# lrjconan/LanczosNetwork

Measured on NVIDIA H100. Metric: QM8 molecules/sec (forward), higher is better.
Workload: dtype f32

## Files before the change

lanczosnetwork_b200/csrc/filter_mlp_chain.cu:

```cuda
#include "tc_gemm.cuh"

namespace {

constexpr int S0MAX = 8;

struct ChainPolicy {
  static constexpr int kStagesB = 2;
  static constexpr int kStagesA = 4;
  struct Params {
    const float* table;
    const int32_t* rowmap;
    const int32_t* nrows;
    const float* W_hi;
    const float* W_lo;
    const float* bias_all;
    float* coeff;
    int Rall, L, S, Hd;
    int dbg;
  };
  static __device__ __forceinline__ bool mma0(const Params& p) { return p.S > S0MAX; }
  static __device__ __forceinline__ int first_stage(const Params& p) { return mma0(p) ? 0 : 1; }
  static __device__ __forceinline__ int steps_per_item(const Params& p) { return mma0(p) ? 4 : 2; }
  static __device__ __forceinline__ int rows(const Params& p) { return p.nrows ? __ldg(p.nrows) : p.Rall; }
  static __device__ __forceinline__ int ntile(const Params& p) { return (rows(p) + tcg::BM - 1) / tcg::BM; }
  static __device__ __forceinline__ void item_range(const Params& p, int cta, int ncta, int& first,
                                                    int& count) {
    const int items = ntile(p) * p.L, base = items / ncta, rem = items % ncta;
    count = base + (cta < rem ? 1 : 0);
    first = cta * base + min(cta, rem);
  }
  static __device__ __forceinline__ int num_steps(const Params& p, int cta, int ncta) {
    int first, count;
    item_range(p, cta, ncta, first, count);
    return count * steps_per_item(p);
  }
  static __device__ __forceinline__ void decode(const Params& p, int cta, int ncta, int it,
                                                int& m_tile, int& sub) {
    const int per = steps_per_item(p), nt = ntile(p);
    int first, count;
    item_range(p, cta, ncta, first, count);
    const int item = first + it / per;
    m_tile = item % nt;
    sub = (item / nt) * 4 + first_stage(p) + it % per;
  }
  static __device__ __forceinline__ int num_kblocks(const Params& p, int sub) {
    return (sub & 3) == 0 ? 1 : p.Hd / tcg::BK;
  }
  static __device__ __forceinline__ int w_row0(const Params& p, int layer, int stage) {
    return layer * (3 * p.Hd + p.S) + stage * p.Hd;
  }
  static __device__ __forceinline__ void w_coords(const Params& p, int sub, int kb, int& col0, int& row0) {
    col0 = kb * tcg::BK;
    row0 = w_row0(p, sub >> 2, sub & 3);
  }
  static __device__ __forceinline__ bool operand_from_acc(const Params& p, int sub) {
    return (sub & 3) > first_stage(p);
  }
  static __device__ __forceinline__ float acc_operand(const Params&, const uint8_t* policy_smem, int sub, int col,
                                                      float x) {
    const float* bs = reinterpret_cast<const float*>(policy_smem) + BS_OFF;
    return fmaxf(x + bs[(sub & 3) * tcg::BN + col], 0.f);
  }

  const Params& p;
  const int tid, r;
  static constexpr int BS_OFF = 2 * tcg::BN * S0MAX;
  float* W1s;
  float* W3s;
  float* bs;
  float* b3s;
  int src, cur_layer;
  float tv[S0MAX];
  float o[S0MAX];

  static size_t smem_bytes() {
    return (BS_OFF + 3 * tcg::BN + S0MAX) * 4;
  }

  __device__ ChainPolicy(const Params& p_, uint8_t* smem, int tid_)
      : p(p_), tid(tid_), r(tid_ & 127), src(-1), cur_layer(-1) {
    W1s = reinterpret_cast<float*>(smem);
    W3s = W1s + tcg::BN * S0MAX;
    bs = W1s + BS_OFF;
    b3s = bs + 3 * tcg::BN;
  }

  __device__ void step_begin(int m_tile, int sub, int, tcg::PhaseTimer& tm) {
    const int layer = sub >> 2;
    if ((sub & 3) != first_stage(p)) return;
    const int i = m_tile * tcg::BM + r;
    src = i < rows(p) ? (p.rowmap ? __ldg(p.rowmap + i) : i) : -1;
    if (layer != cur_layer) {
      tcg::producers_sync<ChainPolicy>();
      const int row0 = w_row0(p, layer, 0), row3 = w_row0(p, layer, 3);
      if (!mma0(p)) {
#pragma unroll 4
        for (int e = tid; e < p.Hd * S0MAX; e += tcg::producer_threads<ChainPolicy>) {
          const int c = e / S0MAX, k = e - c * S0MAX;
          const int64_t o1 = (int64_t)(row0 + c) * p.Hd + k;
          W1s[e] = (k < p.S) ? __ldg(p.W_hi + o1) + __ldg(p.W_lo + o1) : 0.f;
          const int64_t o3 = (int64_t)(row3 + k) * p.Hd + c;
          W3s[e] = (k < p.S) ? __ldg(p.W_hi + o3) + __ldg(p.W_lo + o3) : 0.f;
        }
        if (tid < S0MAX) b3s[tid] = tid < p.S ? __ldg(p.bias_all + row3 + tid) : 0.f;
      }
      for (int e = tid; e < 3 * tcg::BN; e += tcg::producer_threads<ChainPolicy>) {
        const int st = e / tcg::BN, c = e - st * tcg::BN;
        bs[e] = c < p.Hd ? __ldg(p.bias_all + row0 + st * p.Hd + c) : 0.f;
      }
      tcg::producers_sync<ChainPolicy>();
      cur_layer = layer;
      tm.lap(1);
    }
    if (mma0(p)) return;
#pragma unroll
    for (int k = 0; k < S0MAX; ++k)
      tv[k] = (src >= 0 && k < p.S) ? __ldg(p.table + (int64_t)src * p.S + k) : 0.f;
  }

  __device__ __forceinline__ void produce(int sub, int kb, float (&v)[32]) {
    if ((sub & 3) == 0) {
#pragma unroll
      for (int j = 0; j < 32; ++j)
        v[j] = (src >= 0 && j < p.S) ? __ldg(p.table + (int64_t)src * p.S + j) : 0.f;
      return;
    }
#pragma unroll
    for (int j = 0; j < 32; ++j) {
      const int c = kb * tcg::BK + j;
      const float4* wr = reinterpret_cast<const float4*>(W1s + c * S0MAX);
      const float4 wa = wr[0], wb = wr[1];
      float a = bs[c];
      a = fmaf(tv[0], wa.x, a); a = fmaf(tv[1], wa.y, a); a = fmaf(tv[2], wa.z, a); a = fmaf(tv[3], wa.w, a);
      a = fmaf(tv[4], wb.x, a); a = fmaf(tv[5], wb.y, a); a = fmaf(tv[6], wb.z, a); a = fmaf(tv[7], wb.w, a);
      v[j] = fmaxf(a, 0.f);
    }
  }
  __device__ __forceinline__ void pre_epilogue(int) {}
  __device__ __forceinline__ void post_epilogue(int) {}

  __device__ __forceinline__ void store(int sub, int col, const float (&x)[tcg::EW]) {
    const int layer = sub >> 2, stage = sub & 3;
    if (stage == 3) {
      if (src < 0 || col >= p.S) return;
      const float* bias = p.bias_all + w_row0(p, layer, stage);
      float* dst = p.coeff + ((int64_t)layer * p.Rall + src) * p.S;
#pragma unroll
      for (int j = 0; j < tcg::EW; ++j)
        if (col + j < p.S) dst[col + j] = x[j] + __ldg(bias + col + j);
      return;
    }
    if (col >= p.Hd) return;
    const float* b2 = bs + 2 * tcg::BN;
    if (col == 0) {
#pragma unroll
      for (int s = 0; s < S0MAX; ++s) o[s] = 0.f;
    }
#pragma unroll
    for (int j = 0; j < tcg::EW; ++j) {
      const float y = fmaxf(x[j] + b2[col + j], 0.f);
      const float4* wr = reinterpret_cast<const float4*>(W3s + (col + j) * S0MAX);
      const float4 wa = wr[0], wb = wr[1];
      o[0] = fmaf(y, wa.x, o[0]); o[1] = fmaf(y, wa.y, o[1]);
      o[2] = fmaf(y, wa.z, o[2]); o[3] = fmaf(y, wa.w, o[3]);
      o[4] = fmaf(y, wb.x, o[4]); o[5] = fmaf(y, wb.y, o[5]);
      o[6] = fmaf(y, wb.z, o[6]); o[7] = fmaf(y, wb.w, o[7]);
    }
    if (col + tcg::EW < p.Hd || src < 0) return;
    float* dst = p.coeff + ((int64_t)layer * p.Rall + src) * p.S;
#pragma unroll
    for (int s = 0; s < S0MAX; ++s)
      if (s < p.S) dst[s] = o[s] + b3s[s];
  }
};

__global__ void __launch_bounds__(1024)
ritz_rowmap_kernel(const int32_t* __restrict__ gext, int B, int K, int32_t* __restrict__ rowmap,
                   int32_t* __restrict__ nrows) {
  __shared__ int warp_sums[32];
  __shared__ int gbase[1024], gk[1024];
  __shared__ int running;
  const int tid = threadIdx.x, lane = tid & 31, warp = tid >> 5;
  if (tid == 0) running = 0;
  __syncthreads();
  for (int b0 = 0; b0 < B; b0 += 1024) {
    const int b = b0 + tid;
    int k = (b < B) ? min(gext[b * 2 + 1], K) : 0;
    int incl = k;
#pragma unroll
    for (int o = 1; o < 32; o <<= 1) {
      const int t = __shfl_up_sync(0xffffffffu, incl, o);
      if (lane >= o) incl += t;
    }
    if (lane == 31) warp_sums[warp] = incl;
    __syncthreads();
    if (warp == 0) {
      int w = warp_sums[lane], wi = w;
#pragma unroll
      for (int o = 1; o < 32; o <<= 1) {
        const int t = __shfl_up_sync(0xffffffffu, wi, o);
        if (lane >= o) wi += t;
      }
      warp_sums[lane] = wi - w;
    }
    __syncthreads();
    const int base = running + warp_sums[warp] + incl - k;
    gbase[tid] = base;
    gk[tid] = k;
    __syncthreads();
    if (tid == 1023) running = base + k;
    for (int j = warp; j < 1024 && b0 + j < B; j += 32)
      for (int i = lane; i < gk[j]; i += 32) rowmap[gbase[j] + i] = (b0 + j) * K + i;
    __syncthreads();
  }
  if (tid == 0) nrows[0] = running;
}

}

extern "C" {

int lnb_ritz_rowmap(lnb_stream_t stream, const int32_t* gext, int B, int K, int32_t* rowmap,
                    int32_t* nrows) {
  LNB_REQUIRE(gext && rowmap && nrows, "ritz_rowmap: null pointer");
  LNB_REQUIRE(B >= 0 && K >= 1, "ritz_rowmap: bad dims");
  ritz_rowmap_kernel<<<1, 1024, 0, (cudaStream_t)stream>>>(gext, B, K, rowmap, nrows);
  lnb::count_launch();
  return lnb::finish_launch("ritz_rowmap");
}

int lnb_ritz_filter_mlp(lnb_stream_t stream, const float* table, const int32_t* rowmap,
                        const int32_t* nrows, const float* W_hi, const float* W_lo,
                        const float* bias_all, int Rall, int L, int S, int Hd, float* coeff) {
  return lnb_ritz_filter_mlp_ctas(stream, table, rowmap, nrows, W_hi, W_lo, bias_all, Rall, L, S, Hd,
                                  coeff, 0);
}

int lnb_ritz_filter_mlp_ctas(lnb_stream_t stream, const float* table, const int32_t* rowmap,
                             const int32_t* nrows, const float* W_hi, const float* W_lo,
                             const float* bias_all, int Rall, int L, int S, int Hd, float* coeff,
                             int ctas) {
  LNB_REQUIRE(table && W_hi && W_lo && bias_all && coeff, "ritz_filter_mlp: null pointer");
  LNB_REQUIRE((rowmap == nullptr) == (nrows == nullptr), "ritz_filter_mlp: rowmap and nrows go together");
  LNB_REQUIRE(Rall >= 0 && L >= 1 && S >= 1 && Hd >= 1 && ctas >= 0, "ritz_filter_mlp: bad dims");
  if (S > 32 || Hd % 32 != 0 || Hd > tcg::BN) {
    lnb::set_err("ritz_filter_mlp: unsupported shape S=%d hidden=%d (needs S<=32, hidden%%32==0, hidden<=128)", S, Hd);
    return LNB_ERR_UNSUPPORTED;
  }
  if (Rall == 0) return LNB_OK;
  const size_t smem = tcg::core_smem(ChainPolicy::kStagesB, ChainPolicy::kStagesA) + 1024 + ChainPolicy::smem_bytes();
  ChainPolicy::Params p{table, rowmap, nrows, W_hi, W_lo, bias_all, coeff, Rall, L, S, Hd, tcg::debug_flags()};
  return tcg::launch<ChainPolicy>(stream, W_hi, W_lo, L * (3 * Hd + S), Hd, smem, lnb::ceil_div(Rall, tcg::BM) * L, p,
                                  "ritz_filter_mlp", ctas);
}

}
```

lanczosnetwork_b200/csrc/tc_gemm.cuh:

```cuda
#pragma once
#include "common.cuh"
#include "sm90.cuh"
#include <stdlib.h>
#include <type_traits>
#include <utility>

namespace tcg {

constexpr int BM = 128, BN = 128, BK = 32;
constexpr int TILE_B_BYTES = BN * BK * 4;
constexpr int STAGE_B_BYTES = 2 * TILE_B_BYTES;
constexpr int TILE_A_BYTES = BM * BK * 4;
constexpr int STAGE_A_BYTES = 2 * TILE_A_BYTES;
constexpr int EW = 16;
constexpr int CONSUMER_THREADS = 256;
constexpr int CONSUMER_REGS = 168;
constexpr int MAX_B_STAGES = 6, MAX_A_STAGES = 4;

template <class P, class = void> struct ProducerGroups : std::integral_constant<int, 1> {};
template <class P>
struct ProducerGroups<P, std::void_t<decltype(P::kProducerGroups)>> : std::integral_constant<int, P::kProducerGroups> {};
template <class P> constexpr int producer_threads = 128 * ProducerGroups<P>::value;
template <class P> constexpr int cta_threads = producer_threads<P> + CONSUMER_THREADS;
template <class P> constexpr int producer_regs = (65536 - CONSUMER_THREADS * CONSUMER_REGS) / producer_threads<P> / 8 * 8;
__host__ __device__ constexpr int core_smem(int stages_b, int stages_a) {
  return stages_b * STAGE_B_BYTES + stages_a * STAGE_A_BYTES + 256;
}
__host__ __device__ constexpr int pass_cols(int stages_a) {
  return stages_a * STAGE_A_BYTES / (BM * 4) < BN ? stages_a * STAGE_A_BYTES / (BM * 4) : BN;
}

__device__ __forceinline__ uint8_t* a_ring(uint8_t* policy_smem, int stages_b, int stages_a) {
  return policy_smem - core_smem(stages_b, stages_a) + stages_b * STAGE_B_BYTES;
}

struct Core {
  uint8_t* Bst;
  uint8_t* Ast;
  uint64_t* b_full;
  uint64_t* b_empty;
  uint64_t* a_full;
  uint64_t* a_empty;
  uint64_t* stg_full;
  uint64_t* stg_empty;
  uint64_t* kept_read;
};

__device__ __forceinline__ Core carve(uint8_t* base, int stages_b, int stages_a) {
  Core c;
  c.Bst = base;
  c.Ast = base + stages_b * STAGE_B_BYTES;
  uint64_t* bars = reinterpret_cast<uint64_t*>(c.Ast + stages_a * STAGE_A_BYTES);
  c.b_full = bars;
  c.b_empty = c.b_full + MAX_B_STAGES;
  c.a_full = c.b_empty + MAX_B_STAGES;
  c.a_empty = c.a_full + MAX_A_STAGES;
  c.stg_full = c.a_empty + MAX_A_STAGES;
  c.stg_empty = c.stg_full + 1;
  c.kept_read = c.stg_empty + 1;
  return c;
}

__device__ unsigned long long* g_prof = nullptr;

struct PhaseTimer {
  unsigned long long* buf;
  long long t0;
  __device__ __forceinline__ void start(int cta, int tid) {
    buf = (tid == 0 && g_prof) ? g_prof + cta * 32 : nullptr;
    if (buf) t0 = clock64();
  }
  __device__ __forceinline__ void start_if(int cta, bool owner) {
    buf = (owner && g_prof) ? g_prof + cta * 32 : nullptr;
    if (buf) t0 = clock64();
  }
  __device__ __forceinline__ void lap(int slot) {
    if (buf) { long long t = clock64(); atomicAdd(&buf[slot], (unsigned long long)(t - t0)); t0 = t; }
  }
};

template <class Policy>
__device__ __forceinline__ void producers_sync() {
  asm volatile("bar.sync 1, %0;" ::"n"(producer_threads<Policy>) : "memory");
}
__device__ __forceinline__ void consumers_sync() {
  asm volatile("bar.sync 2, %0;" ::"n"(CONSUMER_THREADS) : "memory");
}

__device__ __forceinline__ int stg_index(int row, int col, int pw) {
  return row * pw + ((((col >> 2) ^ row) & (pw / 4 - 1)) << 2) + (col & 3);
}

template <class P, class = void> struct HasAccInit : std::false_type {};
template <class P> struct HasAccInit<P, std::void_t<decltype(&P::acc_init)>> : std::true_type {};
template <class P, class = void> struct HasOperandFromAcc : std::false_type {};
template <class P> struct HasOperandFromAcc<P, std::void_t<decltype(&P::operand_from_acc)>> : std::true_type {};
template <class P>
constexpr bool kScaledProduce =
    std::is_same_v<decltype(std::declval<P&>().produce(0, 0, std::declval<float (&)[32]>())), float>;

template <class Policy>
__device__ __forceinline__ bool next_from_acc(const typename Policy::Params& p, int cta, int ncta, int it,
                                              int nsteps, int& nkb_next) {
  if (it + 1 >= nsteps) return false;
  int m_tile, sub;
  Policy::decode(p, cta, ncta, it + 1, m_tile, sub);
  nkb_next = Policy::num_kblocks(p, sub);
  return Policy::operand_from_acc(p, sub);
}

constexpr int SKIP_MMA = 2;
constexpr int SKIP_TMA = 4;

template <class Policy, int kSkip>
__device__ __forceinline__ void tc_gemm_body(const CUtensorMap& map_hi, const CUtensorMap& map_lo,
                                             const typename Policy::Params& p) {
  extern __shared__ __align__(16) uint8_t smem_raw[];
  const uint32_t pad = (1024u - (sm90::smem_u32(smem_raw) & 1023u)) & 1023u;
  uint8_t* base = smem_raw + pad;
  constexpr int SB = Policy::kStagesB, SA = Policy::kStagesA;
  static_assert(SB >= 1 && SB <= MAX_B_STAGES && SA >= 1 && SA <= MAX_A_STAGES, "ring depths");
  constexpr int PW = pass_cols(SA);
  constexpr int NPASS = BN / PW;
  constexpr bool kAccInit = HasAccInit<Policy>::value;
  static_assert(!kAccInit || NPASS == 1, "a drain kept in the A ring must fit it in one pass");
  constexpr bool kOpAcc = HasOperandFromAcc<Policy>::value;
  constexpr bool kQueue = !kAccInit;
  static_assert(!kOpAcc || SA * BK >= BN, "an operand written from the accumulators needs one A stage per k-block");
  constexpr int NG = ProducerGroups<Policy>::value, PT = producer_threads<Policy>;
  constexpr bool kScaled = kScaledProduce<Policy>;
  static_assert(NG == 1 || (NG == 2 && !kOpAcc && PW % (2 * EW) == 0), "two producer groups: no operand_from_acc");
  Core c = carve(base, SB, SA);
  uint8_t* policy_smem = base + core_smem(SB, SA);
  float* stg = reinterpret_cast<float*>(c.Ast);

  const int tid = threadIdx.x, warp = tid >> 5, lane = tid & 31;
  const int role = __shfl_sync(0xffffffffu, tid / 128, 0);
  const int cta = blockIdx.x, ncta = gridDim.x;
  const int nsteps = __shfl_sync(0xffffffffu, Policy::num_steps(p, cta, ncta), 0);
  unsigned long long prof_ns0 = 0;
  long long prof_c0 = 0;
  if (tid == 0 && g_prof) {
    asm volatile("mov.u64 %0, %globaltimer;" : "=l"(prof_ns0));
    prof_c0 = clock64();
  }

  if (warp == PT / 32 && lane == 0) {
    sm90::tma_prefetch_desc(&map_hi);
    sm90::tma_prefetch_desc(&map_lo);
    for (int s = 0; s < SB; ++s) {
      sm90::mbar_init(&c.b_full[s], 1);
      sm90::mbar_init(&c.b_empty[s], CONSUMER_THREADS / 32);
    }
    for (int s = 0; s < SA; ++s) {
      sm90::mbar_init(&c.a_full[s], PT / NG);
      sm90::mbar_init(&c.a_empty[s], CONSUMER_THREADS / 32);
    }
    sm90::mbar_init(c.stg_full, CONSUMER_THREADS);
    sm90::mbar_init(c.stg_empty, PT);
    sm90::mbar_init(c.kept_read, CONSUMER_THREADS / 32);
    sm90::fence_barrier_init();
  }
  __syncthreads();

  if (NG == 1 ? role == 0 : role < NG) {
    if constexpr (NG > 1) sm90::setmaxnreg_dec<producer_regs<Policy>>();
    const int r = tid & 127;
    const int grp = NG == 1 ? 0 : role;
    Policy pol(p, policy_smem, tid);
    uint32_t cnt = 0;
    uint32_t npass = 0;
    uint32_t nkept = 0;
    bool after_kept = false;
    for (int it = 0; it < nsteps; ++it) {
      int m_tile, sub;
      Policy::decode(p, cta, ncta, it, m_tile, sub);
      int nkb = Policy::num_kblocks(p, sub);
      bool kept = false, to_acc = false;
      if constexpr (kAccInit) kept = Policy::drain_kept(p, sub);
      if constexpr (kOpAcc) {
        if (Policy::operand_from_acc(p, sub)) nkb = 0;
        int nkb_next;
        to_acc = next_from_acc<Policy>(p, cta, ncta, it, nsteps, nkb_next);
      }
      PhaseTimer tm;
      tm.start(cta, tid);
      pol.step_begin(m_tile, sub, NG == 1 ? 0 : (int)((grp + NG - cnt % NG) % NG), tm);
      [[maybe_unused]] float v_kept[32];
      for (int kb = 0; kb < nkb; ++kb, ++cnt) {
        if constexpr (NG > 1) {
          if (cnt % NG != (uint32_t)grp) continue;
        }
        float v[32];
        [[maybe_unused]] float scale = 1.f;
        if (!(p.dbg & 8)) {
          if constexpr (kScaled) scale = pol.produce(sub, kb, v_kept);
          else pol.produce(sub, kb, v);
        }
        const uint32_t sa = cnt % SA;
        if (kAccInit && (NG == 1 ? kb == 0 : kb < NG) && after_kept) {
          sm90::mbar_wait(c.kept_read, nkept & 1u);
          if constexpr (NG == 1) ++nkept;
        }
        sm90::mbar_wait(&c.a_empty[sa], ((cnt / SA) & 1u) ^ 1u);
        if (!(p.dbg & 1)) {
          uint8_t* hi = c.Ast + sa * STAGE_A_BYTES + r * 128;
#pragma unroll
          for (int j = 0; j < 8; ++j) {
            if constexpr (kScaled) {
#pragma unroll
              for (int i = 4 * j; i < 4 * j + 4; ++i) v[i] = __fmul_rn(scale, v_kept[i]);
            }
            uint4 h, l;
            h.x = sm90::tf32_rna_bits(v[4 * j + 0]); h.y = sm90::tf32_rna_bits(v[4 * j + 1]);
            h.z = sm90::tf32_rna_bits(v[4 * j + 2]); h.w = sm90::tf32_rna_bits(v[4 * j + 3]);
            l.x = sm90::tf32_rna_bits(v[4 * j + 0] - __uint_as_float(h.x));
            l.y = sm90::tf32_rna_bits(v[4 * j + 1] - __uint_as_float(h.y));
            l.z = sm90::tf32_rna_bits(v[4 * j + 2] - __uint_as_float(h.z));
            l.w = sm90::tf32_rna_bits(v[4 * j + 3] - __uint_as_float(h.w));
            const int off = (j ^ (r & 7)) * 16;
            *reinterpret_cast<uint4*>(hi + off) = h;
            *reinterpret_cast<uint4*>(hi + TILE_A_BYTES + off) = l;
          }
        }
        sm90::fence_proxy_async();
        sm90::mbar_arrive(&c.a_full[sa]);
      }
      if constexpr (NG > 1) {
        if (kAccInit && after_kept) ++nkept;
      }
      tm.lap((sub & 1) ? 8 : 3);
      pol.pre_epilogue(sub);
      tm.lap(4);
#pragma unroll 1
      for (int q = 0; q < (kept || to_acc ? 0 : NPASS); ++q, ++npass) {
        sm90::mbar_wait(c.stg_full, npass & 1u);
        if (q == 0) tm.lap((sub & 1) ? 9 : 5);
#pragma unroll 1
        for (int col = q * PW + grp * EW; col < (q + 1) * PW; col += NG * EW) {
          float x[EW];
#pragma unroll
          for (int j = 0; j < EW; j += 4) {
            const float4 t = *reinterpret_cast<const float4*>(stg + stg_index(r, col - q * PW + j, PW));
            x[j] = t.x; x[j + 1] = t.y; x[j + 2] = t.z; x[j + 3] = t.w;
          }
          pol.store(sub, col, x);
        }
        sm90::mbar_arrive(c.stg_empty);
      }
      tm.lap(7);
      producers_sync<Policy>();
      pol.post_epilogue(sub);
      tm.lap(10);
      after_kept = kept;
    }
  } else {
    if constexpr (NG > 1) sm90::setmaxnreg_inc<CONSUMER_REGS>();
    const int wg = role - NG;
    const int wq = warp & 3;
    float d[128];
    uint32_t cnt = 0, npass = 0;
    uint32_t nacc = 0;
    bool after_kept = false;
    const int row0 = wg * 64 + wq * 16 + (lane >> 2), cl = 2 * (lane & 3);
    const bool w_issuer = warp == PT / 32;
    int l_it = 0, l_kb = 0, l_nkb = -1, l_sub = 0;
    uint32_t l_cnt = 0;
    auto load_next = [&]() {
      while (l_it < nsteps) {
        if (l_nkb < 0) {
          int mt;
          Policy::decode(p, cta, ncta, l_it, mt, l_sub);
          l_nkb = Policy::num_kblocks(p, l_sub);
        }
        if (l_kb < l_nkb) break;
        ++l_it; l_kb = 0; l_nkb = -1;
      }
      if (l_it >= nsteps) return;
      int col0, row0;
      Policy::w_coords(p, l_sub, l_kb, col0, row0);
      const uint32_t st = l_cnt % SB;
      sm90::mbar_wait_uniform(&c.b_empty[st], ((l_cnt / SB) & 1u) ^ 1u);
      uint8_t* dst = c.Bst + st * STAGE_B_BYTES;
      sm90::tma_load_2d_pair_elected<(kSkip & SKIP_TMA) != 0>(w_issuer, &c.b_full[st], STAGE_B_BYTES, dst, &map_hi,
                                                               dst + TILE_B_BYTES, &map_lo, col0, row0);
      ++l_kb; ++l_cnt;
    };
    auto release = [&](uint32_t sb_rel, bool a_stage, uint32_t sa_rel) {
      sm90::mbar_arrive_pred(&c.a_empty[sa_rel], a_stage && lane == 0);
      sm90::mbar_arrive_pred(&c.b_empty[sb_rel], lane == 0);
      load_next();
    };
    for (int i = 0; i < SB; ++i) load_next();
    for (int it = 0; it < nsteps; ++it) {
      int m_tile, sub;
      Policy::decode(p, cta, ncta, it, m_tile, sub);
      const int nkb = Policy::num_kblocks(p, sub);
      bool kept = false, from_acc = false, to_acc = false;
      int nkb_next = 0;
      if constexpr (kOpAcc) {
        from_acc = Policy::operand_from_acc(p, sub);
        to_acc = next_from_acc<Policy>(p, cta, ncta, it, nsteps, nkb_next);
      }
      if constexpr (kAccInit) {
        kept = Policy::drain_kept(p, sub);
        sm90::wgmma_fence_operand(d);
        if (!Policy::acc_init(p, policy_smem, stg, sub, row0, cl, d)) {
#pragma unroll
          for (int i = 0; i < 128; ++i) d[i] = 0.f;
        }
        if (after_kept) {
          __syncwarp();
          if (lane == 0) sm90::mbar_arrive(c.kept_read);
        }
      } else {
#pragma unroll
        for (int i = 0; i < 128; ++i) d[i] = 0.f;
      }
      sm90::wgmma_fence_operand(d);
      for (int kb = 0; kb < nkb; ++kb, ++cnt) {
        const uint32_t acnt = cnt - nacc;
        const uint32_t sb = cnt % SB, sa = from_acc ? (uint32_t)kb : acnt % SA;
        sm90::mbar_wait_uniform(&c.b_full[sb], (cnt / SB) & 1u);
        if (!from_acc) sm90::mbar_wait_uniform(&c.a_full[sa], (acnt / SA) & 1u);
        if constexpr (!(kSkip & SKIP_MMA)) {
          const uint32_t a_hi = sm90::smem_u32(c.Ast + sa * STAGE_A_BYTES) + wg * 64 * 128;
          const uint32_t a_lo = a_hi + TILE_A_BYTES;
          const uint32_t b = sm90::smem_u32(c.Bst + sb * STAGE_B_BYTES);
          sm90::wgmma_fence_operand(d);
          sm90::wgmma_fence();
#pragma unroll
          for (int k = 0; k < BK / 8; ++k) {
            const uint64_t ah = sm90::wgmma_desc_kmajor_sw128(a_hi + 32 * k);
            const uint64_t wh = sm90::wgmma_desc_kmajor_sw128(b + 32 * k);
            sm90::wgmma_n128(d, ah, wh, 1u);
            sm90::wgmma_n128_hi(d, ah, sm90::wgmma_desc_kmajor_sw128(b + TILE_B_BYTES + 32 * k), 1u);
            sm90::wgmma_n128_hi(d, sm90::wgmma_desc_kmajor_sw128(a_lo + 32 * k), wh, 1u);
          }
          sm90::wgmma_commit();
          if constexpr (kQueue) sm90::wgmma_wait_one();
          else sm90::wgmma_wait_all();
          sm90::wgmma_fence_operand(d);
        }
        if constexpr (kQueue) {
          if (kb > 0) release((cnt - 1) % SB, !from_acc, from_acc ? (uint32_t)(kb - 1) : (acnt - 1) % SA);
        } else {
          release(sb, !from_acc, sa);
        }
      }
      if constexpr (!(kSkip & SKIP_MMA)) {
        sm90::wgmma_wait_all();
        sm90::wgmma_fence_operand(d);
      }
      if (kQueue && nkb > 0)
        release((cnt - 1) % SB, !from_acc, from_acc ? (uint32_t)(nkb - 1) : (cnt - nacc - 1) % SA);
      if (from_acc) nacc += nkb;
      PhaseTimer ctm;
      if (to_acc) ctm.start_if(cta, tid == PT);
      consumers_sync();
      if (to_acc) {
        if constexpr (kOpAcc) {
#pragma unroll
          for (int i = 0; i < 64; i += 2) {
            const int col = 8 * (i / 4) + cl, row = row0 + 8 * ((i / 2) % 2), kb = i / 16;
            if (kb < nkb_next) {
              const float y0 = Policy::acc_operand(p, policy_smem, sub, col, d[i] + d[i + 64]);
              const float y1 = Policy::acc_operand(p, policy_smem, sub, col + 1, d[i + 1] + d[i + 65]);
              uint2 h, l;
              h.x = sm90::tf32_rna_bits(y0); h.y = sm90::tf32_rna_bits(y1);
              l.x = sm90::tf32_rna_bits(y0 - __uint_as_float(h.x));
              l.y = sm90::tf32_rna_bits(y1 - __uint_as_float(h.y));
              uint8_t* dst = c.Ast + kb * STAGE_A_BYTES + row * 128 + (((((col & 31) >> 2) ^ row) & 7) << 4) +
                             (col & 3) * 4;
              *reinterpret_cast<uint2*>(dst) = h;
              *reinterpret_cast<uint2*>(dst + TILE_A_BYTES) = l;
            }
          }
          sm90::fence_proxy_async();
          consumers_sync();
          ctm.lap(14);
        }
      } else {
#pragma unroll
        for (int q = 0; q < NPASS; ++q, npass += kept ? 0 : 1) {
          if (!kept) sm90::mbar_wait(c.stg_empty, (npass & 1u) ^ 1u);
#pragma unroll
          for (int i = 0; i < 64; i += 2) {
            const int col = 8 * (i / 4) + cl, row = row0 + 8 * ((i / 2) % 2);
            if (col >= q * PW && col < (q + 1) * PW)
              *reinterpret_cast<float2*>(stg + stg_index(row, col - q * PW, PW)) =
                  make_float2(d[i] + d[i + 64], d[i + 1] + d[i + 65]);
          }
          if (!kept) sm90::mbar_arrive(c.stg_full);
        }
      }
      if (kept) consumers_sync();
      after_kept = kept;
    }
  }

  __syncthreads();
  if (tid == 0 && g_prof) {
    unsigned long long ns1;
    asm volatile("mov.u64 %0, %globaltimer;" : "=l"(ns1));
    atomicAdd(&g_prof[cta * 32 + 11], ns1 - prof_ns0);
    atomicAdd(&g_prof[cta * 32 + 12], (unsigned long long)(clock64() - prof_c0));
    g_prof[cta * 32 + 13] = prof_ns0;
  }
}

template <class Policy>
__global__ void __launch_bounds__(cta_threads<Policy>, 1)
tc_gemm_kernel(const __grid_constant__ CUtensorMap map_hi,
               const __grid_constant__ CUtensorMap map_lo, const typename Policy::Params p) {
  tc_gemm_body<Policy, 0>(map_hi, map_lo, p);
}

template <class Policy, int kSkip>
__global__ void __launch_bounds__(cta_threads<Policy>, 1)
tc_gemm_probe_kernel(const __grid_constant__ CUtensorMap map_hi,
                     const __grid_constant__ CUtensorMap map_lo, const typename Policy::Params p) {
  tc_gemm_body<Policy, kSkip>(map_hi, map_lo, p);
}

__device__ __forceinline__ void store_row_chunk(float* orow, int ncols, const float* bias, bool relu,
                                                int col, const float (&x)[EW]) {
  if (orow == nullptr || col >= ncols) return;
  const bool vec_ok = (reinterpret_cast<uintptr_t>(orow + col) & 15) == 0;
#pragma unroll
  for (int j = 0; j < EW; j += 4) {
    float o[4];
#pragma unroll
    for (int u = 0; u < 4; ++u) {
      const int n = col + j + u;
      float y = x[j + u];
      if (n < ncols) {
        if (bias) y += __ldg(bias + n);
        if (relu) y = fmaxf(y, 0.f);
      }
      o[u] = y;
    }
    if (vec_ok && col + j + 3 < ncols) {
      *reinterpret_cast<float4*>(orow + col + j) = make_float4(o[0], o[1], o[2], o[3]);
    } else {
#pragma unroll
      for (int u = 0; u < 4; ++u)
        if (col + j + u < ncols) orow[col + j + u] = o[u];
    }
  }
}

typedef CUresult (*EncodeTiledFn)(CUtensorMap*, CUtensorMapDataType, cuuint32_t, void*,
                                  const cuuint64_t*, const cuuint64_t*, const cuuint32_t*,
                                  const cuuint32_t*, CUtensorMapInterleave, CUtensorMapSwizzle,
                                  CUtensorMapL2promotion, CUtensorMapFloatOOBfill);

inline EncodeTiledFn get_encode_fn() {
  static EncodeTiledFn fn = nullptr;
  if (!fn) {
    void* ptr = nullptr;
    cudaDriverEntryPointQueryResult q;
    if (cudaGetDriverEntryPoint("cuTensorMapEncodeTiled", &ptr, cudaEnableDefault, &q) == cudaSuccess &&
        q == cudaDriverEntryPointSuccess)
      fn = reinterpret_cast<EncodeTiledFn>(ptr);
  }
  return fn;
}

inline int make_weight_map(CUtensorMap* map, const float* W, int rows, int cols, const char* who,
                           int box_rows = BN) {
  EncodeTiledFn enc = get_encode_fn();
  if (!enc) { lnb::set_err("%s: cuTensorMapEncodeTiled unavailable", who); return LNB_ERR_UNSUPPORTED; }
  cuuint64_t gdim[2] = {(cuuint64_t)cols, (cuuint64_t)rows};
  cuuint64_t gstride[1] = {(cuuint64_t)cols * sizeof(float)};
  cuuint32_t box[2] = {(cuuint32_t)BK, (cuuint32_t)box_rows};
  cuuint32_t estr[2] = {1, 1};
  CUresult r = enc(map, CU_TENSOR_MAP_DATA_TYPE_FLOAT32, 2, const_cast<float*>(W), gdim, gstride,
                   box, estr, CU_TENSOR_MAP_INTERLEAVE_NONE, CU_TENSOR_MAP_SWIZZLE_128B,
                   CU_TENSOR_MAP_L2_PROMOTION_L2_256B, CU_TENSOR_MAP_FLOAT_OOB_FILL_NONE);
  if (r != CUDA_SUCCESS) {
    lnb::set_err("%s: cuTensorMapEncodeTiled failed (CUresult %d)", who, (int)r);
    return LNB_ERR_ARG;
  }
  return LNB_OK;
}

inline int debug_flags() {
  const char* e = getenv("LNB_DBG");
  return e ? atoi(e) : 0;
}

inline int sm_count() {
  int dev = 0, n = 132;
  if (cudaGetDevice(&dev) == cudaSuccess)
    cudaDeviceGetAttribute(&n, cudaDevAttrMultiProcessorCount, dev);
  return n > 0 ? n : 132;
}

inline int persistent_grid(int items, int max_ctas = 0) {
  int grid = items < sm_count() ? items : sm_count();
  if (max_ctas > 0 && grid > max_ctas) grid = max_ctas;
  const int cap = lnb::debug_max_ctas();
  if (cap > 0 && grid > cap) grid = cap;
  return grid;
}

static unsigned long long* g_prof_mirrored = nullptr;

static int sync_prof_buffer(const char* who) {
  unsigned long long* buf = lnb::prof_buffer();
  if (buf == g_prof_mirrored) return LNB_OK;
  cudaError_t e = cudaMemcpyToSymbol(g_prof, &buf, sizeof(buf));
  if (e != cudaSuccess) { lnb::set_err("%s: %s", who, cudaGetErrorString(e)); return (int)e; }
  g_prof_mirrored = buf;
  return LNB_OK;
}

template <class Pol>
static int launch(lnb_stream_t stream, const float* W_hi, const float* W_lo, int w_rows, int w_cols,
                  size_t smem, int items, const typename Pol::Params& p, const char* who,
                  int max_ctas = 0) {
  CUtensorMap map_hi, map_lo;
  int rc = make_weight_map(&map_hi, W_hi, w_rows, w_cols, who);
  if (rc != LNB_OK) return rc;
  rc = make_weight_map(&map_lo, W_lo, w_rows, w_cols, who);
  if (rc != LNB_OK) return rc;
  rc = sync_prof_buffer(who);
  if (rc != LNB_OK) return rc;
  const int skip = p.dbg & (SKIP_MMA | SKIP_TMA);
  auto kern = skip == 0                    ? tc_gemm_kernel<Pol>
              : skip == SKIP_MMA           ? tc_gemm_probe_kernel<Pol, SKIP_MMA>
              : skip == SKIP_TMA           ? tc_gemm_probe_kernel<Pol, SKIP_TMA>
                                           : tc_gemm_probe_kernel<Pol, SKIP_MMA | SKIP_TMA>;
  cudaFuncSetAttribute(kern, cudaFuncAttributeMaxDynamicSharedMemorySize, (int)smem);
  kern<<<persistent_grid(items, max_ctas), cta_threads<Pol>, smem, (cudaStream_t)stream>>>(map_hi, map_lo, p);
  lnb::count_launch();
  return lnb::finish_launch(who);
}

}
```

Measured before the change: 1.226 million.

## Prefetch next item's first A k-blocks during final-stage drain

Adds an acc_free barrier so the producer can start building the first k-blocks of the next item's first stage while the last stage's results are still being drained. To make this possible the drain staging buffer is moved above the first DS A-ring stages, and the output row index is latched in pre_epilogue so that step_begin for the next item does not overwrite it. The intent is to hide producer latency at item boundaries in the chained MLP. In exchange it adds barrier bookkeeping and ring-index conditions that must hold, or the early path is skipped.

```diff
diff --git a/lanczosnetwork_b200/csrc/filter_mlp_chain.cu b/lanczosnetwork_b200/csrc/filter_mlp_chain.cu
--- a/lanczosnetwork_b200/csrc/filter_mlp_chain.cu
+++ b/lanczosnetwork_b200/csrc/filter_mlp_chain.cu
@@ -7,6 +7,8 @@
 struct ChainPolicy {
   static constexpr int kStagesB = 2;
   static constexpr int kStagesA = 4;
+  static constexpr int kDrainStage = 2;
+  static constexpr int kEarlyKblocks = 2;
   struct Params {
     const float* table;
     const int32_t* rowmap;
@@ -70,6 +72,7 @@
   float* bs;
   float* b3s;
   int src, cur_layer;
+  int src_out;
   float tv[S0MAX];
   float o[S0MAX];
 
@@ -78,7 +81,7 @@
   }
 
   __device__ ChainPolicy(const Params& p_, uint8_t* smem, int tid_)
-      : p(p_), tid(tid_), r(tid_ & 127), src(-1), cur_layer(-1) {
+      : p(p_), tid(tid_), r(tid_ & 127), src(-1), cur_layer(-1), src_out(-1) {
     W1s = reinterpret_cast<float*>(smem);
     W3s = W1s + tcg::BN * S0MAX;
     bs = W1s + BS_OFF;
@@ -136,15 +139,18 @@
       v[j] = fmaxf(a, 0.f);
     }
   }
-  __device__ __forceinline__ void pre_epilogue(int) {}
+  __device__ __forceinline__ int early_kblocks(int sub_next) const {
+    return !mma0(p) && (sub_next >> 2) == cur_layer ? kEarlyKblocks : 0;
+  }
+  __device__ __forceinline__ void pre_epilogue(int) { src_out = src; }
   __device__ __forceinline__ void post_epilogue(int) {}
 
   __device__ __forceinline__ void store(int sub, int col, const float (&x)[tcg::EW]) {
     const int layer = sub >> 2, stage = sub & 3;
     if (stage == 3) {
-      if (src < 0 || col >= p.S) return;
+      if (src_out < 0 || col >= p.S) return;
       const float* bias = p.bias_all + w_row0(p, layer, stage);
-      float* dst = p.coeff + ((int64_t)layer * p.Rall + src) * p.S;
+      float* dst = p.coeff + ((int64_t)layer * p.Rall + src_out) * p.S;
 #pragma unroll
       for (int j = 0; j < tcg::EW; ++j)
         if (col + j < p.S) dst[col + j] = x[j] + __ldg(bias + col + j);
@@ -166,8 +172,8 @@
       o[4] = fmaf(y, wb.x, o[4]); o[5] = fmaf(y, wb.y, o[5]);
       o[6] = fmaf(y, wb.z, o[6]); o[7] = fmaf(y, wb.w, o[7]);
     }
-    if (col + tcg::EW < p.Hd || src < 0) return;
-    float* dst = p.coeff + ((int64_t)layer * p.Rall + src) * p.S;
+    if (col + tcg::EW < p.Hd || src_out < 0) return;
+    float* dst = p.coeff + ((int64_t)layer * p.Rall + src_out) * p.S;
 #pragma unroll
     for (int s = 0; s < S0MAX; ++s)
       if (s < p.S) dst[s] = o[s] + b3s[s];
diff --git a/lanczosnetwork_b200/csrc/tc_gemm.cuh b/lanczosnetwork_b200/csrc/tc_gemm.cuh
--- a/lanczosnetwork_b200/csrc/tc_gemm.cuh
+++ b/lanczosnetwork_b200/csrc/tc_gemm.cuh
@@ -44,6 +44,7 @@
   uint64_t* stg_full;
   uint64_t* stg_empty;
   uint64_t* kept_read;
+  uint64_t* acc_free;
 };
 
 __device__ __forceinline__ Core carve(uint8_t* base, int stages_b, int stages_a) {
@@ -58,6 +59,7 @@
   c.stg_full = c.a_empty + MAX_A_STAGES;
   c.stg_empty = c.stg_full + 1;
   c.kept_read = c.stg_empty + 1;
+  c.acc_free = c.kept_read + 1;
   return c;
 }
 
@@ -95,6 +97,10 @@
 template <class P> struct HasAccInit<P, std::void_t<decltype(&P::acc_init)>> : std::true_type {};
 template <class P, class = void> struct HasOperandFromAcc : std::false_type {};
 template <class P> struct HasOperandFromAcc<P, std::void_t<decltype(&P::operand_from_acc)>> : std::true_type {};
+template <class P, class = void> struct HasEarlyKblocks : std::false_type {};
+template <class P> struct HasEarlyKblocks<P, std::void_t<decltype(&P::early_kblocks)>> : std::true_type {};
+template <class P, class = void> struct DrainStage : std::integral_constant<int, 0> {};
+template <class P> struct DrainStage<P, std::void_t<decltype(P::kDrainStage)>> : std::integral_constant<int, P::kDrainStage> {};
 template <class P>
 constexpr bool kScaledProduce =
     std::is_same_v<decltype(std::declval<P&>().produce(0, 0, std::declval<float (&)[32]>())), float>;
@@ -107,6 +113,23 @@
   Policy::decode(p, cta, ncta, it + 1, m_tile, sub);
   nkb_next = Policy::num_kblocks(p, sub);
   return Policy::operand_from_acc(p, sub);
+}
+
+__device__ __forceinline__ void store_split_row(uint8_t* stage, int r, const float (&v)[32]) {
+  uint8_t* hi = stage + r * 128;
+#pragma unroll
+  for (int j = 0; j < 8; ++j) {
+    uint4 h, l;
+    h.x = sm90::tf32_rna_bits(v[4 * j + 0]); h.y = sm90::tf32_rna_bits(v[4 * j + 1]);
+    h.z = sm90::tf32_rna_bits(v[4 * j + 2]); h.w = sm90::tf32_rna_bits(v[4 * j + 3]);
+    l.x = sm90::tf32_rna_bits(v[4 * j + 0] - __uint_as_float(h.x));
+    l.y = sm90::tf32_rna_bits(v[4 * j + 1] - __uint_as_float(h.y));
+    l.z = sm90::tf32_rna_bits(v[4 * j + 2] - __uint_as_float(h.z));
+    l.w = sm90::tf32_rna_bits(v[4 * j + 3] - __uint_as_float(h.w));
+    const int off = (j ^ (r & 7)) * 16;
+    *reinterpret_cast<uint4*>(hi + off) = h;
+    *reinterpret_cast<uint4*>(hi + TILE_A_BYTES + off) = l;
+  }
 }
 
 constexpr int SKIP_MMA = 2;
@@ -130,9 +153,15 @@
   constexpr int NG = ProducerGroups<Policy>::value, PT = producer_threads<Policy>;
   constexpr bool kScaled = kScaledProduce<Policy>;
   static_assert(NG == 1 || (NG == 2 && !kOpAcc && PW % (2 * EW) == 0), "two producer groups: no operand_from_acc");
+  constexpr bool kEarly = HasEarlyKblocks<Policy>::value;
+  constexpr int DS = DrainStage<Policy>::value;
+  static_assert(DS * STAGE_A_BYTES + BM * PW * 4 <= SA * STAGE_A_BYTES, "the drain must fit the A ring");
+  static_assert(!kEarly || (kOpAcc && NG == 1 && !kAccInit && NPASS == 1 && DS > 0),
+                "early k-blocks: operand_from_acc, one producer group, no acc_init, a one-pass drain above them");
   Core c = carve(base, SB, SA);
   uint8_t* policy_smem = base + core_smem(SB, SA);
   float* stg = reinterpret_cast<float*>(c.Ast);
+  float* drain = reinterpret_cast<float*>(c.Ast + DS * STAGE_A_BYTES);
 
   const int tid = threadIdx.x, warp = tid >> 5, lane = tid & 31;
   const int role = __shfl_sync(0xffffffffu, tid / 128, 0);
@@ -159,6 +188,7 @@
     sm90::mbar_init(c.stg_full, CONSUMER_THREADS);
     sm90::mbar_init(c.stg_empty, PT);
     sm90::mbar_init(c.kept_read, CONSUMER_THREADS / 32);
+    if constexpr (kEarly) sm90::mbar_init(c.acc_free, CONSUMER_THREADS / 32);
     sm90::fence_barrier_init();
   }
   __syncthreads();
@@ -171,23 +201,35 @@
     uint32_t cnt = 0;
     uint32_t npass = 0;
     uint32_t nkept = 0;
+    uint32_t nfree = 0;
+    int early = 0;
     bool after_kept = false;
+    [[maybe_unused]] auto put_early_kblock = [&](int sub, int kb) {
+      float v[32];
+      if (!(p.dbg & 8)) pol.produce(sub, kb, v);
+      const uint32_t sa = cnt % SA;
+      sm90::mbar_wait(&c.a_empty[sa], ((cnt / SA) & 1u) ^ 1u);
+      if (!(p.dbg & 1)) store_split_row(c.Ast + sa * STAGE_A_BYTES, r, v);
+      sm90::fence_proxy_async();
+      sm90::mbar_arrive(&c.a_full[sa]);
+    };
     for (int it = 0; it < nsteps; ++it) {
       int m_tile, sub;
       Policy::decode(p, cta, ncta, it, m_tile, sub);
       int nkb = Policy::num_kblocks(p, sub);
-      bool kept = false, to_acc = false;
+      bool kept = false, to_acc = false, from_acc = false;
       if constexpr (kAccInit) kept = Policy::drain_kept(p, sub);
       if constexpr (kOpAcc) {
-        if (Policy::operand_from_acc(p, sub)) nkb = 0;
+        from_acc = Policy::operand_from_acc(p, sub);
+        if (from_acc) nkb = 0;
         int nkb_next;
         to_acc = next_from_acc<Policy>(p, cta, ncta, it, nsteps, nkb_next);
       }
       PhaseTimer tm;
       tm.start(cta, tid);
-      pol.step_begin(m_tile, sub, NG == 1 ? 0 : (int)((grp + NG - cnt % NG) % NG), tm);
+      if (early == 0) pol.step_begin(m_tile, sub, NG == 1 ? 0 : (int)((grp + NG - cnt % NG) % NG), tm);
       [[maybe_unused]] float v_kept[32];
-      for (int kb = 0; kb < nkb; ++kb, ++cnt) {
+      for (int kb = early; kb < nkb; ++kb, ++cnt) {
         if constexpr (NG > 1) {
           if (cnt % NG != (uint32_t)grp) continue;
         }
@@ -232,6 +274,26 @@
       tm.lap((sub & 1) ? 8 : 3);
       pol.pre_epilogue(sub);
       tm.lap(4);
+      early = 0;
+      if constexpr (kEarly) {
+        if (from_acc && !to_acc) {
+          if (it + 1 < nsteps) {
+            int m_next, sub_next;
+            Policy::decode(p, cta, ncta, it + 1, m_next, sub_next);
+            int e = Policy::operand_from_acc(p, sub_next) ? 0
+                                                          : min(pol.early_kblocks(sub_next), Policy::num_kblocks(p, sub_next));
+            for (int k = 0; k < e; ++k)
+              if ((cnt + k) % SA >= (uint32_t)DS) e = 0;
+            if (e > 0) {
+              sm90::mbar_wait(c.acc_free, nfree & 1u);
+              pol.step_begin(m_next, sub_next, 0, tm);
+              for (; early < e; ++early, ++cnt) put_early_kblock(sub_next, early);
+              tm.lap(6);
+            }
+          }
+          ++nfree;
+        }
+      }
 #pragma unroll 1
       for (int q = 0; q < (kept || to_acc ? 0 : NPASS); ++q, ++npass) {
         sm90::mbar_wait(c.stg_full, npass & 1u);
@@ -241,7 +303,7 @@
           float x[EW];
 #pragma unroll
           for (int j = 0; j < EW; j += 4) {
-            const float4 t = *reinterpret_cast<const float4*>(stg + stg_index(r, col - q * PW + j, PW));
+            const float4 t = *reinterpret_cast<const float4*>(drain + stg_index(r, col - q * PW + j, PW));
             x[j] = t.x; x[j + 1] = t.y; x[j + 2] = t.z; x[j + 3] = t.w;
           }
           pol.store(sub, col, x);
@@ -318,6 +380,10 @@
         for (int i = 0; i < 128; ++i) d[i] = 0.f;
       }
       sm90::wgmma_fence_operand(d);
+      [[maybe_unused]] const int free_kb = from_acc && !to_acc ? min(nkb, DS) : 0;
+      auto free_after = [&](int kb_rel) {
+        if constexpr (kEarly) sm90::mbar_arrive_pred(c.acc_free, kb_rel == free_kb - 1 && lane == 0);
+      };
       for (int kb = 0; kb < nkb; ++kb, ++cnt) {
         const uint32_t acnt = cnt - nacc;
         const uint32_t sb = cnt % SB, sa = from_acc ? (uint32_t)kb : acnt % SA;
@@ -343,17 +409,23 @@
           sm90::wgmma_fence_operand(d);
         }
         if constexpr (kQueue) {
-          if (kb > 0) release((cnt - 1) % SB, !from_acc, from_acc ? (uint32_t)(kb - 1) : (acnt - 1) % SA);
+          if (kb > 0) {
+            release((cnt - 1) % SB, !from_acc, from_acc ? (uint32_t)(kb - 1) : (acnt - 1) % SA);
+            free_after(kb - 1);
+          }
         } else {
           release(sb, !from_acc, sa);
+          free_after(kb);
         }
       }
       if constexpr (!(kSkip & SKIP_MMA)) {
         sm90::wgmma_wait_all();
         sm90::wgmma_fence_operand(d);
       }
-      if (kQueue && nkb > 0)
+      if (kQueue && nkb > 0) {
         release((cnt - 1) % SB, !from_acc, from_acc ? (uint32_t)(nkb - 1) : (cnt - nacc - 1) % SA);
+        free_after(nkb - 1);
+      }
       if (from_acc) nacc += nkb;
       PhaseTimer ctm;
       if (to_acc) ctm.start_if(cta, tid == PT);
@@ -388,7 +460,7 @@
           for (int i = 0; i < 64; i += 2) {
             const int col = 8 * (i / 4) + cl, row = row0 + 8 * ((i / 2) % 2);
             if (col >= q * PW && col < (q + 1) * PW)
-              *reinterpret_cast<float2*>(stg + stg_index(row, col - q * PW, PW)) =
+              *reinterpret_cast<float2*>(drain + stg_index(row, col - q * PW, PW)) =
                   make_float2(d[i] + d[i + 64], d[i + 1] + d[i + 65]);
           }
           if (!kept) sm90::mbar_arrive(c.stg_full);
```

New measurement: 1.218 million, median of 6. Within noise of the previous version (-0.6%).
